# ParsaEsmati/SEA

Measured on AMD Instinct MI355X. Metric: rollout steps/sec (full-context forward, recompute mode) on cylinder_flow-shaped fields, higher is better.
Workload: dtype bf16

## Files before the change

include/sea_hip.h:

```cpp
#ifndef SEA_HIP_H
#define SEA_HIP_H

#include <stddef.h>
#include <stdint.h>

#ifdef __cplusplus
extern "C" {
#endif

#define SEA_ABI_VERSION 8

enum { SEA_F32 = 0, SEA_BF16 = 1 };

enum {
    SEA_OK = 0,
    SEA_EINVAL = -1,
    SEA_ELAUNCH = -2,
    SEA_EUNSUPPORTED = -3
};

int sea_abi_version(void);
const char* sea_last_error(void);
const char* sea_last_form(int* a, int* b);
int sea_struct_sizes(int* out, int cap);
// ... 393 lines not shown
    const float* b3;
    void* mod3;
    int32_t ldw3, ldmod3;
    uint32_t* memo_stamps;
    void* memo_mods;
    const uint32_t* memo_epoch;
    int32_t* memo_count;
    uint32_t* memo_rows;
    int32_t ldmemo, pad_;
} SeaAdalnQkv;
int sea_adaln_qkv(const SeaAdalnQkv* groups, int n_groups, const SeaQkvCommon* common, const SeaGemmGroup* riders, int n_riders, const SeaSiluGroup* silu, int n_silu,
                  const float* silu_c, int silu_M, const SeaIbParams* ib, float eps, int dtype, void* stream);

#define SEA_CHAIN_MAX_PROJ 6
#define SEA_CHAIN_MAX_GROUPS 3
typedef struct {
    const void* att[SEA_XTAIL_MAX_SEG];
    const void* Wp[SEA_XTAIL_MAX_SEG];
    const void* a2;
    const void* W2;
    const float* b2;
    const float* Xin;
    float* X;
    void* Xact;
    int32_t n_seg, ldatt, ldwp, lda2, ldw2, ldxin, ldx, ldxact;
    int32_t M, D, E, has_down, n_proj;
    float bias_scale;
    SeaGemmNormGroup down;
    SeaQkvGroup proj[SEA_CHAIN_MAX_PROJ];
    uint32_t* tile_stamps;
    const float* tile_cond;
    const uint32_t* tile_epoch;
    int32_t* tile_count;
    int32_t tile_sets, pad_;
} SeaRowChain;

int sea_row_chain(const SeaRowChain* params, int n_groups, const SeaQkvCommon* common, float eps, int dtype, void* stream);
struct SeaIbParams_;
int sea_row_chain_riders(const SeaRowChain* params, int n_groups, const SeaQkvCommon* common, const SeaGemmGroup* riders, int n_riders, int tile0, int n_tiles,
                         const struct SeaIbParams_* ib, float eps, int dtype, void* stream);

enum { SEA_OP_GEMM = 1, SEA_OP_QKV = 2, SEA_OP_ATTN = 3, SEA_OP_NORM = 4, SEA_OP_SILU = 5, SEA_OP_IB = 6, SEA_OP_CONVERT = 8, SEA_OP_GEMM_NORM = 9, SEA_OP_XTAIL = 10, SEA_OP_MLP1 = 11, SEA_OP_MLP2 = 13, SEA_OP_GEMM_FEW = 14, SEA_OP_QKV_FEW = 15, SEA_OP_CHAIN = 16, SEA_OP_ADALN = 17, SEA_OP_MLPB = 18, SEA_OP_AQKV = 19, SEA_OP_SPLITK = 20 };
// ... 336 lines not shown
```

sea_amd/_native.py:

```python
from __future__ import annotations

import ctypes as C
import os
from typing import Optional

import torch

_HERE = os.path.dirname(os.path.abspath(__file__))
LIB_PATH = os.path.join(_HERE, "csrc", "libsea_hip.so")

SEA_F32, SEA_BF16 = 0, 1
ABI_VERSION = 8
MAX_GROUPS = 16
CTL_GRAD_NORM, CTL_CLIP, CTL_INV_BC1, CTL_INV_SQRT_BC2, CTL_APPLIED, CTL_STEP, CTL_SKIPPED, CTL_CLIPPED, CTL_WORDS = range(9)
MAX_ATTN_PROBLEMS = 8
MAX_NORM_GROUPS = 16
MAX_SILU_GROUPS = 24

_vp, _i32, _i64, _f32 = C.c_void_p, C.c_int32, C.c_int64, C.c_float


class SeaDropout(C.Structure):
    _fields_ = [("seed", C.c_uint32), ("stream", C.c_uint32), ("thr", _i32), ("mode", _i32)]

# ... 101 lines not shown

XTAIL_MAX_SEG = 4
XTAIL_MAX_GROUPS = 4
MAX_SILU_IB = 4


class SeaExchangeTail(C.Structure):
    _fields_ = [("att", _vp * XTAIL_MAX_SEG), ("Wp", _vp * XTAIL_MAX_SEG), ("Wup", _vp), ("bup", _vp), ("X", _vp), ("Xact", _vp),
                ("n_seg", _i32), ("ldatt", _i32), ("ldwp", _i32), ("ldwup", _i32), ("ldx", _i32), ("ldxact", _i32),
                ("M", _i32), ("D", _i32), ("E", _i32), ("has_down", _i32), ("bias_scale", _f32),
                ("down", SeaGemmNormGroup)]


CHAIN_MAX_PROJ = 6
CHAIN_MAX_GROUPS = 3
CHAIN_MAX_RIDERS = 8


class SeaRowChain(C.Structure):
    _fields_ = [("att", _vp * XTAIL_MAX_SEG), ("Wp", _vp * XTAIL_MAX_SEG), ("a2", _vp), ("W2", _vp), ("b2", _vp), ("Xin", _vp), ("X", _vp), ("Xact", _vp),
                ("n_seg", _i32), ("ldatt", _i32), ("ldwp", _i32), ("lda2", _i32), ("ldw2", _i32), ("ldxin", _i32), ("ldx", _i32), ("ldxact", _i32),
                ("M", _i32), ("D", _i32), ("E", _i32), ("has_down", _i32), ("n_proj", _i32), ("bias_scale", _f32),
                ("down", SeaGemmNormGroup), ("proj", SeaQkvGroup * CHAIN_MAX_PROJ),
                ("tile_stamps", _vp), ("tile_cond", _vp), ("tile_epoch", _vp), ("tile_count", _vp), ("tile_sets", _i32), ("pad_", _i32)]


MAX_ADALN_GROUPS = 16


class SeaAdalnGroup(C.Structure):
    _fields_ = [("A", _vp), ("W", _vp), ("bias", _vp), ("X", _vp), ("gamma", _vp), ("beta", _vp), ("Yact", _vp), ("Y32", _vp), ("mean", _vp), ("rstd", _vp),
                ("lda", _i32), ("ldw", _i32), ("ldx", _i32), ("ldyact", _i32), ("ldy32", _i32), ("M", _i32), ("d", _i32), ("K", _i32)]


MAX_SPLITK_GROUPS = 8


# ... 403 lines not shown
```

sea_amd/csrc/chain.hip:

```cpp
#include "norm_epilogue.hpp"
#include "gemm_tile.hpp"
#include "ib_rows.hpp"
#include <stdlib.h>

struct ChainLaunch {
    SeaRowChain p[SEA_CHAIN_MAX_GROUPS];
    SeaQkvCommon c;
    float eps;
    int n_groups;
    unsigned long long* stamps;
    ChainRiderPod rg[SEA_CHAIN_MAX_RIDERS];
    int n_riders, rider_t0, rider_n, ib_wgs;
    SeaIbParams ib;
};
static_assert(sizeof(ChainLaunch) <= 4096, "kernel arguments of sea_row_chain");

static unsigned long long* g_chain_stamps = nullptr;
extern "C" void sea_chain_debug_stamps(unsigned long long* buf) { g_chain_stamps = buf; }

template <int D, int E, int MI>
struct ChainCfg {
    static constexpr int BM = 16 * MI, BKB = 128, BK = 64;
    static constexpr int KTD = D / BK, KTE = E / BK;
    static constexpr int AT_BYTES = BM * E * 2;
// ... 131 lines not shown
    float* Y32;
    void* Yact;
    float* mean;
    float* rstd;
};

template <int D, int E, int MI>
__global__ __launch_bounds__(256) void row_chain_kernel(const ChainLaunch L) {
    using T = __bf16;
    using C = ChainCfg<D, E, MI>;
    constexpr int BM = C::BM, KTD = C::KTD, KTE = C::KTE, NI1 = C::NI1, NI2 = C::NI2, NI3 = C::NI3, NI4 = C::NI4, SMAX = C::SMAX;
    constexpr int A_KTS = BM * 128;
    extern __shared__ __attribute__((aligned(16))) char smem[];
    const int tid = threadIdx.x, lane = tid & 63, wave = tid >> 6;
    const int r = lane & 15, g = lane >> 4;
    if ((int)blockIdx.y == L.n_groups) {
        const int x = blockIdx.x;
        if (x < L.rider_n) {
            const int tile = L.rider_t0 + x;
            int gi = 0;
            while (gi + 1 < L.n_riders && tile >= L.rg[gi + 1].tile_start) ++gi;
            const ChainRiderPod& R = L.rg[gi];
            ChainRiderGroup G;
            G.A = R.A; G.W = R.W; G.bias = R.bias; G.Cact = R.Cact;
            G.lda = R.lda; G.ldw = R.ldw; G.ldcact = R.ldcact; G.M = R.M; G.N = R.N; G.K = R.K;
            const int t = tile - R.tile_start;
            const int tiles_n = (R.N + 127) / 128;
            const int tm = t / tiles_n, tn = t % tiles_n;
            uint32_t* tst = L.p[0].tile_stamps;
            uint32_t t_c[2] = {0u, 0u}, t_e = 0u;
            int t_row[2] = {-1, -1};
// ... 22 lines not shown
                __syncthreads();
            }
            gemm_tile_body<T, 128, 128, true, true, false>(G, tm, tn, smem, 0);
#pragma unroll
            for (int i = 0; i < 2; ++i)
                if (tst != nullptr && t_row[i] >= 0) reinterpret_cast<uint2*>(tst)[t_row[i]] = make_uint2(t_c[i], t_e);
        } else if (x < L.rider_n + L.ib_wgs) {
            const int row0 = (x - L.rider_n) * 64 + wave * 16;
            for (int i = 0; i < 16; ++i) {
                const int row = row0 + i;
                if (row < L.ib.M) ib_store_row(L.ib, L.ib.c[row], row, lane);
            }
        }
        return;
    }
    ChainParams pl;
    {
        const uint32_t* raw = reinterpret_cast<const uint32_t*>(&L.p[0]) + (size_t)blockIdx.y * (sizeof(SeaRowChain) / 4);
#pragma unroll
        for (int k = 0; k < 4; ++k) {
            const int dw = k * 64 + lane;
            pl.v[k] = dw < (int)(sizeof(SeaRowChain) / 4) ? raw[dw] : 0u;
        }
    }
    const int M = CP_I32(M), S = CP_I32(n_seg);
    const int m0 = blockIdx.x * BM;
    if (m0 >= M) return;
    unsigned long long* stp = L.stamps != nullptr ? L.stamps + (size_t)(blockIdx.y * gridDim.x + blockIdx.x) * 16 : nullptr;
    int stn = 0;
    auto stamp = [&]() {
        if (stp != nullptr && tid == 0 && stn < 16) stp[stn] = wall_clock64();
        ++stn;
    };
    stamp();
    char* AT = smem;
    char* YT = AT + C::AT_BYTES;
    char* WA = YT + C::YT_BYTES;
    char* WB = WA + C::WH_BYTES;
    float* s_rope = reinterpret_cast<float*>(WB + C::WH_BYTES);
    float* s_bias = reinterpret_cast<float*>(reinterpret_cast<char*>(s_rope) + C::ROPE_BYTES);
    float* red = reinterpret_cast<float*>(reinterpret_cast<char*>(s_bias) + C::BIAS_BYTES);
    const unsigned lds0 = __builtin_amdgcn_readfirstlane((unsigned)(uintptr_t)smem);
    const unsigned at_l = lds0, wa_l = lds0 + C::AT_BYTES + C::YT_BYTES, wb_l = wa_l + C::WH_BYTES;
    const int wv = __builtin_amdgcn_readfirstlane(wave);
    const T* W2 = CP_PTR(const T*, W2);
    const int ldw2 = CP_I32(ldw2);
    const bool has_down = CP_I32(has_down) != 0;
    const int n_proj = has_down ? CP_I32(n_proj) : 0;
    const T* Wd = CP_PTR(const T*, down.W);
    const int ldwd = CP_I32(down.ldw);

    if (S > 0) {
        const int ldatt = CP_I32(ldatt), ldwp = CP_I32(ldwp);
#pragma unroll
        for (int s = 0; s < SMAX; ++s) {
            if (s < S) {
                const T* att = reinterpret_cast<const T*>(cp_dyn_u64(pl, CP_DW(att) + 2 * s));
                const T* Wp = reinterpret_cast<const T*>(cp_dyn_u64(pl, CP_DW(Wp) + 2 * s));
                chain_dma_a(att, ldatt, m0, M - 1, BM, KTD, at_l + (unsigned)(s * KTD * A_KTS), wv, lane);
                chain_dma_w(Wp, ldwp, D, 0, KTD, wa_l + (unsigned)(s * D * D * 2), wv, lane);
            }
        }
        chain_dma_w(W2, ldw2, E, 0, KTD, wb_l, wv, lane);
// ... 20 lines not shown
    for (int j = 0; j < NI2; ++j) {
        const int n = wave * (E / 4) + j * 16 + g * 4;
#pragma unroll
        for (int q = 0; q < 4; ++q) bv2[j][q] = 0.f;
        if (b2 != nullptr) load4(b2 + n, bv2[j]);
#pragma unroll
        for (int i = 0; i < MI; ++i) load4(Xin + (int64_t)mrow[i] * ldxin + n, rv2[i][j]);
    }
    ChainNormGroup<D, E> Gd;
    Gd.M = M;
    Gd.bias = CP_PTR(const float*, down.bias);
    Gd.mod = CP_PTR(const void*, down.mod);
    Gd.ldmod = CP_I32(down.ldmod);
    Gd.gamma = CP_PTR(const float*, down.gamma);
    Gd.beta = CP_PTR(const float*, down.beta);
    Gd.Y32 = CP_PTR(float*, down.Y32);
    Gd.ldy32 = CP_I32(down.ldy32);
    Gd.Yact = CP_PTR(void*, down.Yact);
    Gd.ldyact = CP_I32(down.ldyact);
    Gd.mean = CP_PTR(float*, down.mean);
    Gd.rstd = CP_PTR(float*, down.rstd);
    NormEpilogue<T, NI3, true, true, true> epi3[MI];
    if (has_down) {
#pragma unroll
        for (int i = 0; i < MI; ++i) epi3[i].prefetch(Gd, mrow[i], wave * (D / 4), g);
    }
    const int hd = L.c.hd, hd2 = hd >> 1, Tlen = L.c.T, pos0 = L.c.pos0;
    if (n_proj > 0) {
        for (int idx = tid; idx < BM * hd2; idx += 256) {
            const int i = idx / hd2, k = idx - i * hd2;
            int m = m0 + i;
            m = m < M ? m : M - 1;
            const int t = m % Tlen;
            const float2 cs = reinterpret_cast<const float2*>(L.c.rope)[(int64_t)(pos0 + t) * hd2 + k];
            reinterpret_cast<float2*>(s_rope)[idx] = cs;
        }
        int boff = 0;
        for (int e = 0; e < n_proj; ++e) {
            const int base = CP_DW(proj) + e * (int)(sizeof(SeaQkvGroup) / 4);
            const float* bias = reinterpret_cast<const float*>(cp_dyn_u64(pl, base + QK_DW(bias)));
            const int N = (int)cp_dyn_u32(pl, base + QK_DW(N));
            for (int n = tid; n < N; n += 256) s_bias[boff + n] = bias != nullptr ? bias[n] : 0.f;
            boff += N;
        }
    }
#pragma unroll
    for (int j = 0; j < NI2; ++j)
#pragma unroll
        for (int q = 0; q < 4; ++q) {
            touch(bv2[j][q]);
#pragma unroll
            for (int i = 0; i < MI; ++i) touch(rv2[i][j][q]);
        }
// ... 49 lines not shown
                const int kk = wave * (D / 4) + j * 16 + g * 4;
                store4(reinterpret_cast<T*>(YT + (kk >> 6) * A_KTS + (i * 16 + r) * 128 + ((((kk & 63) >> 3) ^ (r & 7)) << 4) + (kk & 7) * 2), gsum[i][j][0], gsum[i][j][1], gsum[i][j][2],
                       gsum[i][j][3]);
            }
        lds_barrier();
        if (has_down) chain_dma_w(Wd, ldwd, D, 0, KTE, wa_l, wv, lane);
        chain_mma<MI, NI2>(YT, A_KTS, WB, E * 128, wave * (E / 4), KTD, NI2, r, g, acc2);
    } else {
        chain_mma<MI, NI2>(AT, A_KTS, WA, E * 128, wave * (E / 4), KTE / 2, NI2, r, g, acc2);
        lds_barrier();
        if (has_down) chain_dma_w(Wd, ldwd, D, 0, KTE, wa_l, wv, lane);
        chain_mma<MI, NI2>(AT + (KTE / 2) * A_KTS, A_KTS, WB, E * 128, wave * (E / 4), KTE / 2, NI2, r, g, acc2);
    }
    lds_barrier();
    stamp();
    int e_next = 0;
    auto burst = [&](unsigned half_l, int& e_lo, int& e_hi) {
        e_lo = e_next;
        int bytes = 0;
        while (e_next < n_proj) {
            const int base = CP_DW(proj) + e_next * (int)(sizeof(SeaQkvGroup) / 4);
            const int N = (int)cp_dyn_u32(pl, base + QK_DW(N));
            if (bytes + N * D * 2 > C::WH_BYTES) break;
            chain_dma_w(reinterpret_cast<const T*>(cp_dyn_u64(pl, base + QK_DW(W))), (int)cp_dyn_u32(pl, base + QK_DW(ldw)), N, 0, KTD, half_l + (unsigned)bytes, wv, lane);
            bytes += N * D * 2;
            ++e_next;
        }
        e_hi = e_next;
    };
    int b_lo[2] = {0, 0}, b_hi[2] = {0, 0};
    if (n_proj > 0) burst(wb_l, b_lo[0], b_hi[0]);
    float v2[MI][NI2][4];
#pragma unroll
    for (int i = 0; i < MI; ++i)
#pragma unroll
        for (int j = 0; j < NI2; ++j) {
            const int n = wave * (E / 4) + j * 16 + g * 4;
#pragma unroll
            for (int q = 0; q < 4; ++q) v2[i][j][q] = acc2[i][j][q] + bv2[j][q] * bias_scale + rv2[i][j][q];
            store4(reinterpret_cast<T*>(AT + (n >> 6) * A_KTS + (i * 16 + r) * 128 + ((((n & 63) >> 3) ^ (r & 7)) << 4) + (n & 7) * 2), v2[i][j][0], v2[i][j][1], v2[i][j][2], v2[i][j][3]);
        }
    asm volatile("s_waitcnt vmcnt(0)" ::: "memory");
    stamp();
    {
        float* X = CP_PTR(float*, X);
        T* Xact = CP_PTR(T*, Xact);
        const int ldx = CP_I32(ldx), ldxact = CP_I32(ldxact);
#pragma unroll
        for (int i = 0; i < MI; ++i) {
            if (!mok[i]) continue;
            float* xr_ = X + (int64_t)(m0 + i * 16 + r) * ldx + wave * (E / 4) + g * 4;
            T* xa_ = Xact != nullptr ? Xact + (int64_t)(m0 + i * 16 + r) * ldxact + wave * (E / 4) + g * 4 : nullptr;
#pragma unroll
            for (int j = 0; j < NI2; ++j) {
                store4(xr_ + j * 16, v2[i][j][0], v2[i][j][1], v2[i][j][2], v2[i][j][3]);
                if (xa_ != nullptr) store4(xa_ + j * 16, v2[i][j][0], v2[i][j][1], v2[i][j][2], v2[i][j][3]);
            }
        }
    }
    stamp();
    if (!has_down) return;
    lds_barrier();
    {
        f32x4 acc3[MI][NI3];
#pragma unroll
        for (int i = 0; i < MI; ++i)
#pragma unroll
            for (int j = 0; j < NI3; ++j) acc3[i][j] = f32x4{0.f, 0.f, 0.f, 0.f};
        chain_mma<MI, NI3>(AT, A_KTS, WA, D * 128, wave * (D / 4), KTE, NI3, r, g, acc3);
#pragma unroll
        for (int i = 0; i < MI; ++i)
            epi3[i].finish(Gd, acc3[i], m0 + i * 16 + r, wave * (D / 4), r, g, wave, L.eps, red + i * 128, n_proj > 0 ? YT + i * 16 * 128 : nullptr, A_KTS);
    }
    stamp();
    if (n_proj == 0) return;
    const int Hh = L.c.H, cap = L.c.cap, Ea = Hh * hd;
    const int hd_sh = 31 - __builtin_clz((unsigned)hd);
    uint32_t offq[MI], offk[MI], offv[MI];
#pragma unroll
    for (int i = 0; i < MI; ++i) {
        const int b_ = mrow[i] / Tlen;
        const int t_ = mrow[i] - b_ * Tlen;
        offq[i] = (uint32_t)((b_ * Hh * Tlen + t_) << hd_sh);
        offk[i] = (uint32_t)((b_ * Hh * cap + pos0 + t_) << hd_sh);
        offv[i] = (uint32_t)(b_ * Hh * hd * cap + pos0 + t_);
    }
    const float q_scale = L.c.q_scale;
    int cur = 0;
    int boff = 0;
    for (;;) {
// ... 129 lines not shown
        R.lda = G.lda; R.ldw = G.ldw; R.ldcact = G.ldcact; R.M = G.M; R.N = G.N; R.K = G.K;
        R.tile_start = rider_total;
        rider_total += ((G.M + 127) / 128) * ((G.N + 127) / 128);
    }
    SEA_REQUIRE(tile0 + n_tiles <= rider_total, "sea_row_chain_riders: tiles [%d, %d) of %d", tile0, tile0 + n_tiles, rider_total);
    L.n_riders = n_riders; L.rider_t0 = tile0; L.rider_n = n_tiles;
    if (ib != nullptr) {
        SEA_REQUIRE(ib->X[0] && ib->c && ib->w1 && ib->M >= 1 && ib->E >= 4 && ib->E % 4 == 0 && ib->ldx >= ib->E && ib->mode >= 0 && ib->mode <= 2 &&
                        (ib->mode != 0 || (ib->b1 && ib->lnw && ib->lnb && ib->w2 && ib->b2 && ib->h >= 1 && ib->h <= 64)),
                    "sea_row_chain_riders: bad info-bottleneck rider");
        L.ib = *ib;
        L.ib_wgs = (ib->M + 63) / 64;
    }
    const int D = params[0].D, E = params[0].E;
    int m_max = 0, any_proj = 0;
    for (int gi = 0; gi < n_groups; ++gi) {
        const SeaRowChain& P = params[gi];
        const bool shape_ok = (P.D == 128 && P.E == 256) || (P.D == 64 && P.E == 128);
        if (dtype != SEA_BF16 || !shape_ok || P.n_seg < 0 || P.n_seg * P.D > P.E) {
            sea_set_error("sea_row_chain: unsupported dtype / shape (dtype=%d D=%d E=%d n_seg=%d): bf16, (D,E) in {(128,256),(64,128)}, n_seg*D <= E", dtype, P.D, P.E, P.n_seg);
            return SEA_EUNSUPPORTED;
        }
        SEA_REQUIRE(P.D == D && P.E == E, "sea_row_chain[%d]: the groups of a launch share their widths", gi);
        SEA_REQUIRE(P.M >= 1 && P.W2 && P.Xin && P.X && sea_aligned16(P.W2) && sea_aligned16(P.b2) && sea_aligned16(P.Xin) && sea_aligned16(P.X) && sea_aligned16(P.Xact),
                    "sea_row_chain[%d]: null / misaligned pointer", gi);
        const int K2 = P.n_seg > 0 ? P.D : P.E;
        SEA_REQUIRE(P.ldw2 % 8 == 0 && P.ldw2 >= K2 && P.ldxin % 4 == 0 && P.ldxin >= P.E && P.ldx % 4 == 0 && P.ldx >= P.E && (!P.Xact || (P.ldxact % 4 == 0 && P.ldxact >= P.E)),
                    "sea_row_chain[%d]: bad strides", gi);
        if (P.n_seg == 0) SEA_REQUIRE(P.a2 && sea_aligned16(P.a2) && P.lda2 % 8 == 0 && P.lda2 >= P.E, "sea_row_chain[%d]: a2: null / misaligned / short rows", gi);
        else SEA_REQUIRE(P.ldatt % 8 == 0 && P.ldatt >= P.D && P.ldwp % 8 == 0 && P.ldwp >= P.D, "sea_row_chain[%d]: bad segment strides", gi);
// ... 17 lines not shown
            const SeaQkvGroup& Q = P.proj[e];
            SEA_REQUIRE(common != nullptr, "sea_row_chain: projections need the SeaQkvCommon");
            const int Ea = common->H * common->hd;
            SEA_REQUIRE(Q.W && sea_aligned16(Q.W) && sea_aligned16(Q.bias) && Q.ldw % 8 == 0 && Q.ldw >= P.D && Q.K == P.D && (Q.N == P.D / 2 || Q.N == P.D || Q.N == 2 * P.D) && Q.N % 64 == 0,
                        "sea_row_chain[%d]: projection %d: W [N, D] with N in {D, 2D} (multiples of 64), K = D (N=%d K=%d ldw=%d)", gi, e, Q.N, Q.K, Q.ldw);
            SEA_REQUIRE((Q.N == P.D && Q.col0 == 0) || (Q.N == 2 * P.D && Q.col0 == P.D), "sea_row_chain[%d]: projection %d: a q entry (N = D, col0 = 0) or a k | v entry (N = 2 D, col0 = D), not N=%d col0=%d", gi, e, Q.N, Q.col0);
            SEA_REQUIRE(Q.col0 >= 0 && Q.col0 % 16 == 0 && Q.col0 + Q.N <= 3 * Ea && Ea == P.D, "sea_row_chain[%d]: projection %d: columns [%d,%d) outside [0,%d) / H hd != D", gi, e, Q.col0, Q.col0 + Q.N, 3 * Ea);
            const bool hasq = Q.col0 < Ea, hask = Q.col0 < 2 * Ea && Q.col0 + Q.N > Ea, hasv = Q.col0 + Q.N > 2 * Ea;
            SEA_REQUIRE((!hasq || Q.Qout) && (!hask || Q.Kout) && (!hasv || Q.Vtout) && sea_aligned16(Q.Qout) && sea_aligned16(Q.Kout) && sea_aligned16(Q.Vtout) && sea_aligned16(Q.Vout),
                        "sea_row_chain[%d]: projection %d: missing / misaligned output pointer", gi, e);
            nsum += Q.N;
            any_proj = 1;
        }
        SEA_REQUIRE(nsum * 4 <= 4096, "sea_row_chain[%d]: the projections' output columns sum to %d (at most 1024)", gi, nsum);
        m_max = P.M > m_max ? P.M : m_max;
    }
    if (any_proj) {
        const SeaQkvCommon& c = *common;
        if (c.hd < 16 || (c.hd & (c.hd - 1)) != 0) {
            sea_set_error("sea_row_chain: unsupported head dim %d (a power of two >= 16: a 16-column block of a projection lies inside one head)", c.hd);
            return SEA_EUNSUPPORTED;
        }
        SEA_REQUIRE(c.rope != nullptr && c.H >= 1 && c.hd >= 4 && c.hd % 4 == 0 && c.T >= 1 && c.pos0 >= 0 && c.cap >= c.pos0 + c.T && m_max % c.T == 0,
                    "sea_row_chain: bad common H=%d hd=%d T=%d pos0=%d cap=%d (M=%d)", c.H, c.hd, c.T, c.pos0, c.cap, m_max);
        SEA_REQUIRE((int64_t)(m_max / c.T + 1) * c.H * c.cap * c.hd < ((int64_t)1 << 31) && (int64_t)(c.pos0 + c.T) * (c.hd / 2) < ((int64_t)1 << 30),
                    "sea_row_chain: attention tensors too large for 32-bit element offsets");
        L.c = c;
    }
    const int forced = sea_tune("chain_rows", 0);
    int mi = ((m_max + 15) / 16) * n_groups <= 256 ? 1 : 2;
    if (forced == 16) mi = 1;
    if (forced == 32) mi = 2;
    if (any_proj && 16 * mi * (L.c.hd / 2) * 8 > 2048) {
        if (mi == 2 && 16 * (L.c.hd / 2) * 8 <= 2048) mi = 1;
        else {
            sea_set_error("sea_row_chain: head dim %d: the rotary rows of a workgroup do not fit their LDS block", L.c.hd);
            return SEA_EUNSUPPORTED;
        }
    }
    hipStream_t s = static_cast<hipStream_t>(stream);
    const int chain_x = (m_max + 16 * mi - 1) / (16 * mi), rider_x = L.rider_n + L.ib_wgs;
    const dim3 grid(chain_x > rider_x ? chain_x : rider_x, n_groups + (rider_x > 0 ? 1 : 0));
    constexpr int rider_lds = GemmMainloop<__bf16, 128, 128>::DMA_LDS_BYTES;
#define LAUNCH_CH(DD, EE, MM)                                                                                   \
    do {                                                                                                        \
        constexpr int own_ = ChainCfg<DD, EE, MM>::LDS_BYTES;                                                   \
        constexpr int max_ = own_ > rider_lds ? own_ : rider_lds;                                               \
        static int once = set_lds_chain(row_chain_kernel<DD, EE, MM>, max_);                                    \
        (void)once;                                                                                             \
        row_chain_kernel<DD, EE, MM><<<grid, dim3(256), (L.rider_n > 0 ? max_ : own_), s>>>(L);                 \
    } while (0)
    if (L.p[0].tile_stamps != nullptr && L.rider_n > 0) {
        const SeaRowChain& P0 = L.p[0];
        SEA_REQUIRE(P0.tile_cond && P0.tile_epoch && P0.tile_sets >= rider_total && ((uintptr_t)P0.tile_stamps & 7) == 0 && ((uintptr_t)P0.tile_cond & 3) == 0 &&
                        ((uintptr_t)P0.tile_epoch & 3) == 0 && ((uintptr_t)P0.tile_count & 3) == 0,
                    "sea_row_chain_riders: tile memo: null / misaligned pointer, or %d stamp sets for %d tiles", P0.tile_sets, rider_total);
        for (int i = 1; i < n_riders; ++i) SEA_REQUIRE(riders[i].M == riders[0].M, "sea_row_chain_riders: tile memo: the rider groups share their rows (one condition per row)");
        if (sea_tune("memo_count", 0) == 0) L.p[0].tile_count = nullptr;
    } else {
        L.p[0].tile_stamps = nullptr;
    }
    if (D == 128) { if (mi == 1) LAUNCH_CH(128, 256, 1); else LAUNCH_CH(128, 256, 2); }
    else { if (mi == 1) LAUNCH_CH(64, 128, 1); else LAUNCH_CH(64, 128, 2); }
#undef LAUNCH_CH
    SEA_CHECK_LAUNCH("sea_row_chain");
    sea_note_form(mi == 1 ? "chain.rows16" : "chain.rows32", L.rider_n, L.ib_wgs);
    return SEA_OK;
}
```

sea_amd/engine.py:

```python
from __future__ import annotations

import os

import ctypes as C
import re
from typing import Dict, List, Optional, Tuple

import torch

from . import _native as N
from . import _switches
from . import ops
from . import ptrcheck
from .plan_forms import INFERENCE, resolve_forms

_QKV = re.compile(r"^(.*\.)(k|q|v)\.(weight|bias)$")
_QKV_RANK = {("q", "weight"): 0, ("k", "weight"): 1, ("v", "weight"): 2, ("q", "bias"): 3, ("k", "bias"): 4, ("v", "bias"): 5}


_BIND_KEYS = {"X_is_x": ("_x_patches", "X"), "R_is_x": ("_x_patches", "R"), "Xin_is_x": ("_x_patches", "Xin"), "Y_is_out": ("_out_patches", "Y32"),
              "dY_is_dout": ("_dout_patches", "dY")}


KV_NO_POOL = ("sea_amd: the KV-cache rollout does not cover exchange_mode='pool' (its sinusoidal positions are relative to the window); "
              "use the recompute rollout")
KV_NO_IB_ATTENTION = ("sea_amd: the KV-cache rollout does not cover ib_addition_mode='attention' (every row attends to the info-bottleneck rows "
                      "of ALL positions of the window, later ones included: rows already produced change as the window grows); use the recompute rollout")
KV_NO_SRC_LEN = "sea_amd: the KV-cache rollout is exact only for src_len == 0; use the recompute rollout (rollout(..., mode='recompute'))"

# ... 588 lines not shown
            nd_old = [self._buf(M, D) for _ in range(F)]
            nd_new = [self._buf(M, D) for _ in range(F)]
            Qc = [self._buf(B, H, T, hd_c) for _ in range(max(F - 1, 1))]
            Qc2 = [[self._buf(B, H, T, hd_c) for _ in range(F - 1)] for _ in range(F)] if chain else None
            Kc = [[[self._buf(B, H, cap, hd_c, zero=True) for _ in range(F)] for _ in range(F)] for _ in range(self.L)]
            Vc = [[[self._buf(B, H, hd_c, cap, zero=True) for _ in range(F)] for _ in range(F)] for _ in range(self.L)]
            att_c = [self._buf(M, D) for _ in range(max(F - 1, 1))]
            gp = self._buf(max(F - 1, 1), M, D)
        pad = fm.hidden_pad
        hbuf = [self._buf(M, S + pad)[:, :S] for _ in range(F)]
        hg = [self._buf(M, S + pad)[:, :S] for _ in range(F)]
        self.ws = dict(xr=xr, xa=xa, n_e=n_e, att_e=att_e, hbuf=hbuf, hg=hg)
        self.kv = dict(Ks=Ks, Vs=Vs, Kc=(Kc if xmode == "sea" else None), Vc=(Vc if xmode == "sea" else None))

        xm = [self._buf(M, E) for _ in range(F)] if lanes else xa
        first = True
        for l in range(self.L):
            pre = f"blocks.{l}."
            last = l == self.L - 1
            if first and not eng.model.add_info_after_cross and (has_ib or ib_attn or concat):
                for i in range(F):
                    rec = _Rec(L.sea_convert_f32_to_act, [None, FE, xr[i].data_ptr(), E, M, Eo, N.SEA_F32], "x.copy")
                    self._x_patches.append((rec.args, 0, i * Eo * 4))
                    self.records.append(rec)
                first = False
            if concat:
                if self._zero_ib is None:
                    self._zero_ib = self._buf(M, self.ib_dim, dtype=f32, zero=True)
                for i in range(F):
                    self._cur.append(self._rec(L.sea_convert_f32_to_act, [self._zero_ib.data_ptr(), self.ib_dim, xr[i][:, Eo:].data_ptr(), E, M, self.ib_dim, N.SEA_F32],
# ... 48 lines not shown
            if chain:
                groups = []
                for i in range(F):
                    proj = []
                    for s_, j in enumerate([j for j in range(F) if j != i]):
                        ca = f"{pre}cross_attn.{i}.{j}."
                        proj.append(dict(W=P.act(ca + "q.weight"), bias=P.f32_vec(ca + "q.bias"), col0=0, Q=Qc2[i][s_]))
                    for a in range(i):
                        ca = f"{pre}cross_attn.{a}.{i}."
                        proj.append(dict(W=P.act(ca + "k.weight", 2 * D), bias=P.f32_vec(ca + "k.bias", 2 * D), col0=D, K=Kc[l][a][i], Vt=Vc[l][a][i]))
                    g = dict(a2=att_e[i], W2=P.act(f"{pre}attn.self.{i}.projection.weight"), Xin=xr[i], X=xr[i], proj=proj,
                             down=dict(W=P.act(f"{pre}cross_down.{i}.weight"), bias=P.f32_vec(f"{pre}cross_down.{i}.bias"), **self._norm_params(f"{pre}ln_cross.{i}.")))
                    if first:
                        g.update(ldxin=FE, Xin_is_x=i * Eo * 4)
                    groups.append(g)
                self._chain(groups, rope_c, hd_c, "self.out_proj_down_qkv")
            else:
                (self._gemm_few if few else self._gemm)(groups, "self.out_proj")
            first = False
            if not cond_joined:
                self._join(1)
                cond_joined = True
            if xmode == "addition":
                ndall = self._buf(F, M, D)
                self._down_norm(pre, range(F), xa, dn, ndall, "add")
                sg = self._buf(M, D)
                self._gemm([dict(A=ndall[0], W=eng.eye(D), n_seg=F, a_seg_stride=M * D, Cact=sg, act=1)], "add.sum_gelu")
                self._gemm([dict(A=sg, W=P.act(f"{pre}cross_up.{i}.weight"), bias=P.f32_vec(f"{pre}cross_up.{i}.bias"), R=xr[i], C32=xr[i])
                            for i in range(F)], "add.up")
            if xmode == "pool":
                FD = F * D
# ... 42 lines not shown
                              bias_scale=float(F - 1), n_seg=F - 1, a_seg_stride=M * D, R=xr[i], C32=xr[i], Cact=(xa[i] if i < F - 1 else None))
                    (self._gemm_few if F == 2 else self._gemm)([up], f"cross{i}.up_sum")
                    if i < F - 1:
                        self._gemm_few([dict(A=xa[i], W=P.act(f"{pre}cross_down.{i}.weight"), bias=P.f32_vec(f"{pre}cross_down.{i}.bias"), C32=dn[i])], f"cross{i}.down_new")
            elif F > 1 and xmode == "sea" and chain:
                for i in range(F):
                    others = [j for j in range(F) if j != i]
                    self._attn([dict(Q=Qc2[i][s_], K=Kc[l][i][j], Vt=Vc[l][i][j], O=att_c[s_]) for s_, j in enumerate(others)], hd_c, D, f"cross{i}.attention")
                    proj = []
                    for b_ in range(i + 1, F):
                        ca = f"{pre}cross_attn.{b_}.{i}."
                        proj.append(dict(W=P.act(ca + "k.weight", 2 * D), bias=P.f32_vec(ca + "k.bias", 2 * D), col0=D, K=Kc[l][b_][i], Vt=Vc[l][b_][i]))
                    down = None
                    if i < F - 1:
                        down = dict(W=P.act(f"{pre}cross_down.{i}.weight"), bias=P.f32_vec(f"{pre}cross_down.{i}.bias"), **self._norm_params(f"{pre}ln_cross.{i}."))
                    self._chain([dict(att=[att_c[s_] for s_ in range(len(others))], Wp=[P.act(f"{pre}cross_attn.{i}.{j}.projection.weight") for j in others],
                                      W2=P.act(f"{pre}cross_up.{i}.weight"), b2=P.f32_vec(f"{pre}cross_up.{i}.bias"), bias_scale=float(F - 1), Xin=xr[i], X=xr[i],
                                      down=down, proj=proj)], rope_c, hd_c, f"cross{i}.tail")
            elif F > 1 and xmode == "sea":
                self._down_norm(pre, range(F), xa, dn, nd_old, "cross", "_old")
                for i in range(F):
                    others = [j for j in range(F) if j != i]
                    qkv_groups, probs, proj_groups = [], [], []
                    for s, j in enumerate(others):
                        src = nd_new[j] if j < i else nd_old[j]
                        ca = f"{pre}cross_attn.{i}.{j}."
                        qkv_groups.append(dict(A=nd_old[i], W=P.act(ca + "q.weight"), bias=P.f32_vec(ca + "q.bias"), col0=0, Q=Qc[s]))
                        qkv_groups.append(dict(A=src, W=P.act(ca + "k.weight", 2 * D), bias=P.f32_vec(ca + "k.bias", 2 * D), col0=D,
                                               K=Kc[l][i][j], Vt=Vc[l][i][j]))
                        probs.append(dict(Q=Qc[s], K=Kc[l][i][j], Vt=Vc[l][i][j], O=att_c[s]))
                        proj_groups.append(dict(A=att_c[s], W=P.act(ca + "projection.weight"), Cact=gp[s], act=1))
                    self._qkv(qkv_groups, rope_c, hd_c, f"cross{i}.qkv_rope")
                    self._attn(probs, hd_c, D, f"cross{i}.attention")
# ... 453 lines not shown
            for k, r in enumerate(recs):
                rc = r.fn(*r.args, stream)
                if rc != 0:
                    N.check(rc, r.name)
                evs[k + 1].record()
            torch.cuda.synchronize()
            for k in range(n):
                tot[k] += evs[k].elapsed_time(evs[k + 1])
        return [(r.name, t / iters) for r, t in zip(recs, tot)]


def blk_pe(eng: "TemporalEngine", layer: int) -> torch.Tensor:
    return eng.model.blocks[layer].pos_encoder.pe[0].to(device=eng.device, dtype=torch.float32)


def _require_gpu(device: torch.device) -> None:
    if device.type != "cuda":
        raise RuntimeError("sea_amd: TemporalModel runs only on an MI355X (no CPU fallback)")


class TemporalEngine:

    def __init__(self, model: torch.nn.Module, device: torch.device, act_dtype: torch.dtype):
        N.lib()
        _require_gpu(device)
        m = model
        self.ib_mode = {"mlp": 0, "linear": 1, "fourier": 2}.get(m.ib_scale_mode.lower(), -1)
        if (m.exchange_mode not in ("sea", "addition", "simple", "pool") or self.ib_mode < 0 or m.ib_addition_mode.lower() not in ("add", "none", "attention", "concat")
                or (self.ib_mode == 0 and m.ib_mlp_layers != 1) or m.ib_num != 1 or (self.ib_mode != 0 and m.embed_dim % 8 and m.ib_addition_mode.lower() != "concat")):
            raise NotImplementedError(
# ... 278 lines not shown
```

sea_amd/ops.py:

```python
from __future__ import annotations

import ctypes as C
import math
from typing import Dict, Optional, Sequence

import torch

from . import _native as N


def _mat(t: torch.Tensor, name: str) -> torch.Tensor:
    N.require_gpu(t, name)
    if t.dim() != 2 or t.stride(1) != 1:
        raise ValueError(f"{name}: need a 2-D tensor with unit inner stride, got shape {tuple(t.shape)} strides {t.stride()}")
    return t


def fill_gemm_group(g: N.SeaGemmGroup, A, W, bias=None, R=None, C32=None, Cact=None, n_seg=1, a_seg_stride=0, act=0,
                    bias_scale=1.0, M=None, N_=None, K=None, Z=None, silu=None, drop=None, ldr=None, ldc32=None) -> None:
    if silu is not None:
        c = silu.get("c")
        g.silu_c, g.silu_w1, g.silu_b1 = N.ptr(c), silu["w1"].data_ptr(), silu["b1"].data_ptr()
        A, R, Z, n_seg, a_seg_stride, act = None, None, None, 1, 0, 0
        M = c.numel() if M is None else M
# ... 302 lines not shown
            fill_silu_group(g, gd["w1"], gd["b1"], gd["Hid"])
    ibp = None
    if ib is not None:
        ibp = N.SeaIbParams()
        fill_ib_params(ibp, **ib)
    N.check(N.lib().sea_adaln_qkv(arr, len(groups), C.byref(c), rarr, len(riders), sarr, len(silu), (silu_c.data_ptr() if silu_c is not None else None),
                                  (silu_c.numel() if silu_c is not None else 0), (C.byref(ibp) if ibp is not None else None), eps, N.dtype_code(dtype), N.stream_ptr()),
            "sea_adaln_qkv")


def row_chain_supported(dtype: torch.dtype, D: int, E: int, n_seg: int, hd: int) -> bool:
    return dtype == torch.bfloat16 and (D, E) in ((128, 256), (64, 128)) and 0 <= n_seg and n_seg * D <= E and hd in (16, 32)


def fill_row_chain(P: N.SeaRowChain, W2, Xin, X, att: Sequence[torch.Tensor] = (), Wp: Sequence[torch.Tensor] = (), a2=None, b2=None, bias_scale: float = 1.0, Xact=None,
                   down: Optional[Dict] = None, proj: Sequence[Dict] = (), ldxin: Optional[int] = None, tile_memo: Optional[Dict] = None) -> None:
    if tile_memo is not None:
        st = tile_memo["stamps"]
        if st.dtype != torch.int32 or st.dim() != 3 or tuple(st.shape[1:]) != (128, 2) or not st.is_contiguous():
            raise ValueError(f"row_chain tile memo: stamps {tuple(st.shape)} {st.dtype}: int32 [tiles, 128, 2], one set per rider tile")
        P.tile_stamps, P.tile_sets = st.data_ptr(), st.shape[0]
        P.tile_cond, P.tile_epoch, P.tile_count = N.ptr(tile_memo.get("cond")), tile_memo["epoch"].data_ptr(), N.ptr(tile_memo.get("count"))
    for s_, a in enumerate(att):
        P.att[s_] = a.data_ptr()
        P.Wp[s_] = Wp[s_].data_ptr()
    P.n_seg = len(att)
    if att:
        P.ldatt, P.ldwp = att[0].stride(0), Wp[0].stride(0)
    if a2 is not None:
        P.a2, P.lda2 = a2.data_ptr(), a2.stride(0)
    P.W2, P.ldw2, P.b2, P.bias_scale = W2.data_ptr(), W2.stride(0), N.ptr(b2), bias_scale
# ... 1458 lines not shown
```

sea_amd/plan_forms.py:

```python
from __future__ import annotations

from dataclasses import dataclass, field
from typing import Dict, Optional, Tuple

import torch

from . import _native as N
from . import _switches
from . import ops

INFERENCE, TRAINING, CONDITION = "inference", "training", "condition"


@dataclass(frozen=True)
class PlanForms:
    lanes: bool
    split_cond: bool
    chain: bool
    riders: bool
    rider_caps: Optional[Tuple[int, ...]]
    gen_a: bool
    fold_ib: bool
    hoist_ib: bool
    ib_rows_here: bool
# ... 2 lines not shown
    few_fold_ln: bool
    hidden_pad: int
    front_chain: bool
    front3: bool
    adaln_front: bool
    front_big: bool
    mlp_fc1: bool
    mlp_norm_in: bool
    mlp_block: bool
    mlp_fc2_proj: bool
    down_norm: bool
    proj_norm: bool
    splitk: bool
    cond_memo: bool = field(default=False, compare=False)
    rider_memo: bool = field(default=False, compare=False)

    @property
    def one_launch_front(self) -> bool:
        return self.front_big or self.front_chain


def resolve_forms(model, B: int, T: int, mode: str, dt: torch.dtype, kind: str = INFERENCE, hoisted: bool = False, hoisted_ib: bool = False,
                  plan_switches: Optional[Dict[str, str]] = None, kv_switches: Optional[Dict[str, str]] = None) -> PlanForms:
    assert kind in (INFERENCE, TRAINING, CONDITION)
    sw = (_switches.parse("SEA_PLAN") if plan_switches is None else plan_switches).get
    kvsw = (_switches.parse("SEA_KV") if kv_switches is None else kv_switches).get
    inference = kind == INFERENCE
    F, H, L = model.num_variables, model.n_heads, model.num_layers
    Eo, E, D, S, M = model.embed_dim, model.internal_embed_dim, model.down_dim, model.mlp_hidden, B * T
    xmode, ib_add = model.exchange_mode, model.ib_addition_mode.lower()
    has_ib, ib_attn, concat = ib_add == "add", ib_add == "attention", ib_add == "concat"
    after, adaln = bool(model.add_info_after_cross), model.LN_type.lower() == "adaln"

    lane_mode = sw("lanes", "auto") if inference and xmode == "sea" and has_ib else "none"
# ... 32 lines not shown
    w1, wn, w2 = sw("mlp1", "auto"), sw("mlpnorm", "auto"), sw("mlp2", "auto")
    mlp_fc1 = inference and w1 != "0" and (w1 == "1" or M >= 1024) and mlp_ok
    mlp_norm_in = mlp_fc1 and (wn == "1" or (wn == "auto" and M <= 4096))
    mlp_block = (mlp_fc1 and inference and (w2 == "1" or (w2 == "auto" and 1024 <= M)) and mlp_ok and Eo == E and sw("mlpblock", "1") != "0")
    if mlp_block:
        mlp_norm_in = mlp_norm_in or (M > 4096 and wn != "0")
    mlp_fc2_proj = not mlp_block and inference and (w2 == "1" or (w2 == "auto" and 1024 <= M <= 4096)) and mlp_ok and Eo == E

    return PlanForms(
        lanes=lanes, split_cond=split_cond, chain=chain, riders=riders, rider_caps=(tuple(int(v) for v in caps.split(":")) if caps else None),
        gen_a=gen_a, fold_ib=fold_ib or hoist_ib, hoist_ib=hoist_ib, ib_rows_here=ib_rows_here, xtail=xtail, few=few, few_fold_ln=S <= 8192,
        hidden_pad=(64 if inference and S % 1024 == 0 else 0), front_chain=front_chain, front3=front3, adaln_front=adaln_front, front_big=front_big,
        mlp_fc1=mlp_fc1, mlp_norm_in=mlp_norm_in, mlp_block=mlp_block, mlp_fc2_proj=mlp_fc2_proj,
        down_norm=(fuse_norm if inference else kind == TRAINING and sw("norm", "1") != "0") and D <= 256 and D % 16 == 0,
        proj_norm=fuse_norm and Eo <= 256 and Eo % 16 == 0 and Eo == E and sw("projnorm", "1") != "0", splitk=sw("splitk", "1") != "0",
        cond_memo=front_chain and riders and sw("cond_memo", "1") != "0", rider_memo=front_chain and riders and sw("rider_memo", "1") != "0")
```

sea_amd/ptrcheck.py:

```python
from __future__ import annotations

import ctypes as C
import os
from typing import Iterable, Iterator, List, Optional, Tuple

import torch

from . import _native as N

_HOST_STRUCTS = (N.SeaLaunchRec, N.SeaStepPatch)


def always() -> bool:
    return os.environ.get("SEA_CHECK_PTRS", "0") == "1"


class Ranges:

    def __init__(self) -> None:
        self._r: List[Tuple[int, int, str]] = []

    def add_tensor(self, t: Optional[torch.Tensor], label: str) -> None:
        if t is None or not isinstance(t, torch.Tensor) or not t.is_cuda or t.numel() == 0:
            return
# ... 234 lines not shown
            roots.append(r.keep)
        for root in roots:
            for st in _walk_structs(root):
                for path, p in iter_pointers(st, type(st).__name__):
                    n += 1
                    if ranges.find(p) is None:
                        raise RuntimeError(f"sea_amd pointer audit ({what}): launch '{r.name}': {path} = {p:#x} lies in no buffer this plan knows "
                                           "(stale address, unpatched field or a tensor that was freed)")
                for field, p, nbytes in _extents(st, esz):
                    if not p:
                        continue
                    hit = ranges.find(p)
                    if hit is not None and nbytes > 0 and p + nbytes > hit[1]:
                        raise RuntimeError(f"sea_amd pointer audit ({what}): launch '{r.name}': {type(st).__name__}.{field} = {p:#x} + {nbytes} bytes runs "
                                           f"{p + nbytes - hit[1]} bytes past the end of its buffer ({hit[2]})")
        for field, p, nbytes in _raw_extents(r, esz):
            hit = ranges.find(p)
            if hit is not None and nbytes > 0 and p + nbytes > hit[1]:
                raise RuntimeError(f"sea_amd pointer audit ({what}): launch '{r.name}': argument {field} = {p:#x} + {nbytes} bytes runs "
                                   f"{p + nbytes - hit[1]} bytes past the end of its buffer ({hit[2]})")
        for a in r.args:
            if isinstance(a, int) and a >= (1 << 32) and ranges.find(a) is None and r.fn is not None and r.name not in ("",):
                if _looks_like_device_pointer(a):
                    raise RuntimeError(f"sea_amd pointer audit ({what}): launch '{r.name}': raw argument {a:#x} lies in no buffer this plan knows")
    return n


def _looks_like_device_pointer(a: int) -> bool:
    return a >= (1 << 40) and a % 4 == 0
```

Measured before the change: 5650.

## Split row-chain projection bursts across sibling workgroup rows to fill CUs

Adds a per-group split factor to the row-chain kernel. Each group's QKV projection bursts are divided among several virtual grid rows. Siblings recompute the shared out-proj and down-norm front, but only the primary writes the residual and norm outputs, so the grid can cover more CUs when the tile count is small. This duplicates front work and needs a separate X buffer per split group (ping-pong allocation), with host and pointer-audit checks that X and Xin do not overlap.

```diff
diff --git a/include/sea_hip.h b/include/sea_hip.h
--- a/include/sea_hip.h
+++ b/include/sea_hip.h
@@ -431,6 +431,7 @@
 
 #define SEA_CHAIN_MAX_PROJ 6
 #define SEA_CHAIN_MAX_GROUPS 3
+#define SEA_CHAIN_MAX_SPLIT 3
 typedef struct {
     const void* att[SEA_XTAIL_MAX_SEG];
     const void* Wp[SEA_XTAIL_MAX_SEG];
@@ -443,6 +444,7 @@
     int32_t n_seg, ldatt, ldwp, lda2, ldw2, ldxin, ldx, ldxact;
     int32_t M, D, E, has_down, n_proj;
     float bias_scale;
+    int32_t split, pad0_;
     SeaGemmNormGroup down;
     SeaQkvGroup proj[SEA_CHAIN_MAX_PROJ];
     uint32_t* tile_stamps;
diff --git a/sea_amd/_native.py b/sea_amd/_native.py
--- a/sea_amd/_native.py
+++ b/sea_amd/_native.py
@@ -139,6 +139,7 @@
 
 CHAIN_MAX_PROJ = 6
 CHAIN_MAX_GROUPS = 3
+CHAIN_MAX_SPLIT = 3
 CHAIN_MAX_RIDERS = 8
 
 
@@ -146,6 +147,7 @@
     _fields_ = [("att", _vp * XTAIL_MAX_SEG), ("Wp", _vp * XTAIL_MAX_SEG), ("a2", _vp), ("W2", _vp), ("b2", _vp), ("Xin", _vp), ("X", _vp), ("Xact", _vp),
                 ("n_seg", _i32), ("ldatt", _i32), ("ldwp", _i32), ("lda2", _i32), ("ldw2", _i32), ("ldxin", _i32), ("ldx", _i32), ("ldxact", _i32),
                 ("M", _i32), ("D", _i32), ("E", _i32), ("has_down", _i32), ("n_proj", _i32), ("bias_scale", _f32),
+                ("split", _i32), ("pad0_", _i32),
                 ("down", SeaGemmNormGroup), ("proj", SeaQkvGroup * CHAIN_MAX_PROJ),
                 ("tile_stamps", _vp), ("tile_cond", _vp), ("tile_epoch", _vp), ("tile_count", _vp), ("tile_sets", _i32), ("pad_", _i32)]
 
diff --git a/sea_amd/csrc/chain.hip b/sea_amd/csrc/chain.hip
--- a/sea_amd/csrc/chain.hip
+++ b/sea_amd/csrc/chain.hip
@@ -3,11 +3,14 @@
 #include "ib_rows.hpp"
 #include <stdlib.h>
 
+#define SEA_CHAIN_MAX_VROWS (SEA_CHAIN_MAX_GROUPS * SEA_CHAIN_MAX_SPLIT)
 struct ChainLaunch {
     SeaRowChain p[SEA_CHAIN_MAX_GROUPS];
     SeaQkvCommon c;
     float eps;
     int n_groups;
+    int n_vrows;
+    uint32_t vrow[SEA_CHAIN_MAX_VROWS];
     unsigned long long* stamps;
     ChainRiderPod rg[SEA_CHAIN_MAX_RIDERS];
     int n_riders, rider_t0, rider_n, ib_wgs;
@@ -169,7 +172,7 @@
     extern __shared__ __attribute__((aligned(16))) char smem[];
     const int tid = threadIdx.x, lane = tid & 63, wave = tid >> 6;
     const int r = lane & 15, g = lane >> 4;
-    if ((int)blockIdx.y == L.n_groups) {
+    if ((int)blockIdx.y == L.n_vrows) {
         const int x = blockIdx.x;
         if (x < L.rider_n) {
             const int tile = L.rider_t0 + x;
@@ -222,9 +225,12 @@
         }
         return;
     }
+    const uint32_t vrow = L.vrow[blockIdx.y];
+    const bool primary = ((vrow >> 8) & 0xffu) == 0u;
+    const int e_first = (int)((vrow >> 16) & 0xffu);
     ChainParams pl;
     {
-        const uint32_t* raw = reinterpret_cast<const uint32_t*>(&L.p[0]) + (size_t)blockIdx.y * (sizeof(SeaRowChain) / 4);
+        const uint32_t* raw = reinterpret_cast<const uint32_t*>(&L.p[0]) + (size_t)(vrow & 0xffu) * (sizeof(SeaRowChain) / 4);
 #pragma unroll
         for (int k = 0; k < 4; ++k) {
             const int dw = k * 64 + lane;
@@ -254,7 +260,7 @@
     const T* W2 = CP_PTR(const T*, W2);
     const int ldw2 = CP_I32(ldw2);
     const bool has_down = CP_I32(has_down) != 0;
-    const int n_proj = has_down ? CP_I32(n_proj) : 0;
+    const int n_proj = has_down ? (int)(vrow >> 24) : 0;
     const T* Wd = CP_PTR(const T*, down.W);
     const int ldwd = CP_I32(down.ldw);
 
@@ -305,19 +311,19 @@
     Gd.ldmod = CP_I32(down.ldmod);
     Gd.gamma = CP_PTR(const float*, down.gamma);
     Gd.beta = CP_PTR(const float*, down.beta);
-    Gd.Y32 = CP_PTR(float*, down.Y32);
+    Gd.Y32 = primary ? CP_PTR(float*, down.Y32) : nullptr;
     Gd.ldy32 = CP_I32(down.ldy32);
-    Gd.Yact = CP_PTR(void*, down.Yact);
+    Gd.Yact = primary ? CP_PTR(void*, down.Yact) : nullptr;
     Gd.ldyact = CP_I32(down.ldyact);
-    Gd.mean = CP_PTR(float*, down.mean);
-    Gd.rstd = CP_PTR(float*, down.rstd);
+    Gd.mean = primary ? CP_PTR(float*, down.mean) : nullptr;
+    Gd.rstd = primary ? CP_PTR(float*, down.rstd) : nullptr;
     NormEpilogue<T, NI3, true, true, true> epi3[MI];
     if (has_down) {
 #pragma unroll
         for (int i = 0; i < MI; ++i) epi3[i].prefetch(Gd, mrow[i], wave * (D / 4), g);
     }
     const int hd = L.c.hd, hd2 = hd >> 1, Tlen = L.c.T, pos0 = L.c.pos0;
-    if (n_proj > 0) {
+    if (n_proj > e_first) {
         for (int idx = tid; idx < BM * hd2; idx += 256) {
             const int i = idx / hd2, k = idx - i * hd2;
             int m = m0 + i;
@@ -327,7 +333,7 @@
             reinterpret_cast<float2*>(s_rope)[idx] = cs;
         }
         int boff = 0;
-        for (int e = 0; e < n_proj; ++e) {
+        for (int e = e_first; e < n_proj; ++e) {
             const int base = CP_DW(proj) + e * (int)(sizeof(SeaQkvGroup) / 4);
             const float* bias = reinterpret_cast<const float*>(cp_dyn_u64(pl, base + QK_DW(bias)));
             const int N = (int)cp_dyn_u32(pl, base + QK_DW(N));
@@ -407,7 +413,7 @@
     }
     lds_barrier();
     stamp();
-    int e_next = 0;
+    int e_next = e_first;
     auto burst = [&](unsigned half_l, int& e_lo, int& e_hi) {
         e_lo = e_next;
         int bytes = 0;
@@ -422,7 +428,7 @@
         e_hi = e_next;
     };
     int b_lo[2] = {0, 0}, b_hi[2] = {0, 0};
-    if (n_proj > 0) burst(wb_l, b_lo[0], b_hi[0]);
+    if (n_proj > e_first) burst(wb_l, b_lo[0], b_hi[0]);
     float v2[MI][NI2][4];
 #pragma unroll
     for (int i = 0; i < MI; ++i)
@@ -435,7 +441,7 @@
         }
     asm volatile("s_waitcnt vmcnt(0)" ::: "memory");
     stamp();
-    {
+    if (primary) {
         float* X = CP_PTR(float*, X);
         T* Xact = CP_PTR(T*, Xact);
         const int ldx = CP_I32(ldx), ldxact = CP_I32(ldxact);
@@ -463,10 +469,10 @@
         chain_mma<MI, NI3>(AT, A_KTS, WA, D * 128, wave * (D / 4), KTE, NI3, r, g, acc3);
 #pragma unroll
         for (int i = 0; i < MI; ++i)
-            epi3[i].finish(Gd, acc3[i], m0 + i * 16 + r, wave * (D / 4), r, g, wave, L.eps, red + i * 128, n_proj > 0 ? YT + i * 16 * 128 : nullptr, A_KTS);
+            epi3[i].finish(Gd, acc3[i], m0 + i * 16 + r, wave * (D / 4), r, g, wave, L.eps, red + i * 128, n_proj > e_first ? YT + i * 16 * 128 : nullptr, A_KTS);
     }
     stamp();
-    if (n_proj == 0) return;
+    if (n_proj == e_first) return;
     const int Hh = L.c.H, cap = L.c.cap, Ea = Hh * hd;
     const int hd_sh = 31 - __builtin_clz((unsigned)hd);
     uint32_t offq[MI], offk[MI], offv[MI];
@@ -626,6 +632,7 @@
     }
     const int D = params[0].D, E = params[0].E;
     int m_max = 0, any_proj = 0;
+    int split_max = 1, split_asked = 0, n_vrows = 0;
     for (int gi = 0; gi < n_groups; ++gi) {
         const SeaRowChain& P = params[gi];
         const bool shape_ok = (P.D == 128 && P.E == 256) || (P.D == 64 && P.E == 128);
@@ -673,7 +680,35 @@
         }
         SEA_REQUIRE(nsum * 4 <= 4096, "sea_row_chain[%d]: the projections' output columns sum to %d (at most 1024)", gi, nsum);
         m_max = P.M > m_max ? P.M : m_max;
-    }
+        SEA_REQUIRE(P.split >= 0 && P.split <= SEA_CHAIN_MAX_SPLIT, "sea_row_chain[%d]: split=%d (0 .. %d)", gi, P.split, SEA_CHAIN_MAX_SPLIT);
+        int burst_end[SEA_CHAIN_MAX_PROJ], n_bursts = 0;
+        for (int e = 0, bytes = 0; e < P.n_proj; ++e) {
+            const int eb = P.proj[e].N * P.D * 2;
+            if (n_bursts == 0 || bytes + eb > P.E * P.D * 2) {
+                ++n_bursts;
+                bytes = 0;
+            }
+            bytes += eb;
+            burst_end[n_bursts - 1] = e + 1;
+        }
+        int sp = P.split > 1 ? P.split : 1;
+        split_asked |= P.split > 1 ? 1 : 0;
+        sp = sp > n_bursts ? (n_bursts > 0 ? n_bursts : 1) : sp;
+        if (sp > 1) {
+            const char *xi = reinterpret_cast<const char*>(P.Xin), *xo = reinterpret_cast<const char*>(P.X);
+            const int64_t xi_bytes = ((int64_t)(P.M - 1) * P.ldxin + P.E) * 4, xo_bytes = ((int64_t)(P.M - 1) * P.ldx + P.E) * 4;
+            SEA_REQUIRE(xi + xi_bytes <= xo || xo + xo_bytes <= xi,
+                        "sea_row_chain[%d]: split=%d needs X and Xin in distinct memory (a sibling may read its residual rows after sibling 0 has stored the updated ones)", gi, P.split);
+        }
+        for (int k = 0, b0 = 0; k < sp; ++k) {
+            const int nb = n_bursts / sp + (k >= sp - n_bursts % sp ? 1 : 0);
+            const int e_lo = sp == 1 ? 0 : (b0 == 0 ? 0 : burst_end[b0 - 1]), e_hi = sp == 1 ? P.n_proj : burst_end[b0 + nb - 1];
+            L.vrow[n_vrows++] = (uint32_t)gi | (uint32_t)k << 8 | (uint32_t)e_lo << 16 | (uint32_t)e_hi << 24;
+            b0 += nb;
+        }
+        split_max = sp > split_max ? sp : split_max;
+    }
+    L.n_vrows = n_vrows;
     if (any_proj) {
         const SeaQkvCommon& c = *common;
         if (c.hd < 16 || (c.hd & (c.hd - 1)) != 0) {
@@ -687,7 +722,7 @@
         L.c = c;
     }
     const int forced = sea_tune("chain_rows", 0);
-    int mi = ((m_max + 15) / 16) * n_groups <= 256 ? 1 : 2;
+    int mi = ((m_max + 15) / 16) * n_vrows <= 256 ? 1 : 2;
     if (forced == 16) mi = 1;
     if (forced == 32) mi = 2;
     if (any_proj && 16 * mi * (L.c.hd / 2) * 8 > 2048) {
@@ -699,7 +734,7 @@
     }
     hipStream_t s = static_cast<hipStream_t>(stream);
     const int chain_x = (m_max + 16 * mi - 1) / (16 * mi), rider_x = L.rider_n + L.ib_wgs;
-    const dim3 grid(chain_x > rider_x ? chain_x : rider_x, n_groups + (rider_x > 0 ? 1 : 0));
+    const dim3 grid(chain_x > rider_x ? chain_x : rider_x, n_vrows + (rider_x > 0 ? 1 : 0));
     constexpr int rider_lds = GemmMainloop<__bf16, 128, 128>::DMA_LDS_BYTES;
 #define LAUNCH_CH(DD, EE, MM)                                                                                   \
     do {                                                                                                        \
@@ -723,6 +758,7 @@
     else { if (mi == 1) LAUNCH_CH(64, 128, 1); else LAUNCH_CH(64, 128, 2); }
 #undef LAUNCH_CH
     SEA_CHECK_LAUNCH("sea_row_chain");
-    sea_note_form(mi == 1 ? "chain.rows16" : "chain.rows32", L.rider_n, L.ib_wgs);
+    if (split_asked) sea_note_form("chain.split", split_max, 0);
+    else sea_note_form(mi == 1 ? "chain.rows16" : "chain.rows32", L.rider_n, L.ib_wgs);
     return SEA_OK;
 }
diff --git a/sea_amd/engine.py b/sea_amd/engine.py
--- a/sea_amd/engine.py
+++ b/sea_amd/engine.py
@@ -12,7 +12,7 @@
 from . import _switches
 from . import ops
 from . import ptrcheck
-from .plan_forms import INFERENCE, resolve_forms
+from .plan_forms import CHAIN_SPLIT_GROWTH, INFERENCE, chain_bursts, chain_splits, resolve_forms
 
 _QKV = re.compile(r"^(.*\.)(k|q|v)\.(weight|bias)$")
 _QKV_RANK = {("q", "weight"): 0, ("k", "weight"): 1, ("v", "weight"): 2, ("q", "bias"): 3, ("k", "bias"): 4, ("v", "bias"): 5}
@@ -631,6 +631,30 @@
         self.kv = dict(Ks=Ks, Vs=Vs, Kc=(Kc if xmode == "sea" else None), Vc=(Vc if xmode == "sea" else None))
 
         xm = [self._buf(M, E) for _ in range(F)] if lanes else xa
+        cus = device_cu_count() if fm.chain_split else 0
+        spare: List[torch.Tensor] = []
+
+        def split_chain(groups: List[dict], fields) -> List[dict]:
+            if not fm.chain_split or cus <= 0:
+                return groups
+            n, t16 = len(groups), (M + 15) // 16
+            rows = 16 if t16 * n <= 256 else 32
+            sp = chain_splits([chain_bursts([q["W"].shape[0] for q in g["proj"]], D, E) for g in groups], [(M + rows - 1) // rows] * n, cus,
+                              max_growth=(None if fm.chain_split_all else CHAIN_SPLIT_GROWTH))
+            if rows == 16 and t16 * sum(sp) > 256:
+                return groups
+            out, freed = [], []
+            for g, i, s_ in zip(groups, fields, sp):
+                if s_ > 1:
+                    g = dict(g, split=s_)
+                    if "Xin_is_x" not in g:
+                        new = spare.pop() if spare else self._buf(M, E, dtype=f32)
+                        freed.append(xr[i])
+                        g["X"] = xr[i] = new
+                out.append(g)
+            spare.extend(freed)
+            return out
+
         first = True
         for l in range(self.L):
             pre = f"blocks.{l}."
@@ -709,7 +733,7 @@
                     if first:
                         g.update(ldxin=FE, Xin_is_x=i * Eo * 4)
                     groups.append(g)
-                self._chain(groups, rope_c, hd_c, "self.out_proj_down_qkv")
+                self._chain(split_chain(groups, range(F)), rope_c, hd_c, "self.out_proj_down_qkv")
             else:
                 (self._gemm_few if few else self._gemm)(groups, "self.out_proj")
             first = False
@@ -782,9 +806,10 @@
                     down = None
                     if i < F - 1:
                         down = dict(W=P.act(f"{pre}cross_down.{i}.weight"), bias=P.f32_vec(f"{pre}cross_down.{i}.bias"), **self._norm_params(f"{pre}ln_cross.{i}."))
-                    self._chain([dict(att=[att_c[s_] for s_ in range(len(others))], Wp=[P.act(f"{pre}cross_attn.{i}.{j}.projection.weight") for j in others],
-                                      W2=P.act(f"{pre}cross_up.{i}.weight"), b2=P.f32_vec(f"{pre}cross_up.{i}.bias"), bias_scale=float(F - 1), Xin=xr[i], X=xr[i],
-                                      down=down, proj=proj)], rope_c, hd_c, f"cross{i}.tail")
+                    tail = dict(att=[att_c[s_] for s_ in range(len(others))], Wp=[P.act(f"{pre}cross_attn.{i}.{j}.projection.weight") for j in others],
+                                W2=P.act(f"{pre}cross_up.{i}.weight"), b2=P.f32_vec(f"{pre}cross_up.{i}.bias"), bias_scale=float(F - 1), Xin=xr[i], X=xr[i],
+                                down=down, proj=proj)
+                    self._chain(split_chain([tail], [i]), rope_c, hd_c, f"cross{i}.tail")
             elif F > 1 and xmode == "sea":
                 self._down_norm(pre, range(F), xa, dn, nd_old, "cross", "_old")
                 for i in range(F):
@@ -1268,6 +1293,11 @@
     return eng.model.blocks[layer].pos_encoder.pe[0].to(device=eng.device, dtype=torch.float32)
 
 
+def device_cu_count() -> int:
+    n = C.c_int(0)
+    return n.value if N.lib().sea_device_info(C.byref(n), None, 0) == 0 else 0
+
+
 def _require_gpu(device: torch.device) -> None:
     if device.type != "cuda":
         raise RuntimeError("sea_amd: TemporalModel runs only on an MI355X (no CPU fallback)")
diff --git a/sea_amd/ops.py b/sea_amd/ops.py
--- a/sea_amd/ops.py
+++ b/sea_amd/ops.py
@@ -340,7 +340,8 @@
 
 
 def fill_row_chain(P: N.SeaRowChain, W2, Xin, X, att: Sequence[torch.Tensor] = (), Wp: Sequence[torch.Tensor] = (), a2=None, b2=None, bias_scale: float = 1.0, Xact=None,
-                   down: Optional[Dict] = None, proj: Sequence[Dict] = (), ldxin: Optional[int] = None, tile_memo: Optional[Dict] = None) -> None:
+                   down: Optional[Dict] = None, proj: Sequence[Dict] = (), ldxin: Optional[int] = None, tile_memo: Optional[Dict] = None, split: int = 1) -> None:
+    P.split = split
     if tile_memo is not None:
         st = tile_memo["stamps"]
         if st.dtype != torch.int32 or st.dim() != 3 or tuple(st.shape[1:]) != (128, 2) or not st.is_contiguous():
diff --git a/sea_amd/plan_forms.py b/sea_amd/plan_forms.py
--- a/sea_amd/plan_forms.py
+++ b/sea_amd/plan_forms.py
@@ -1,7 +1,7 @@
 from __future__ import annotations
 
 from dataclasses import dataclass, field
-from typing import Dict, Optional, Tuple
+from typing import Dict, List, Optional, Sequence, Tuple
 
 import torch
 
@@ -40,10 +40,39 @@
     splitk: bool
     cond_memo: bool = field(default=False, compare=False)
     rider_memo: bool = field(default=False, compare=False)
+    chain_split: bool = field(default=False, compare=False)
+    chain_split_all: bool = field(default=False, compare=False)
 
     @property
     def one_launch_front(self) -> bool:
         return self.front_big or self.front_chain
+
+
+def chain_bursts(widths: Sequence[int], D: int, E: int) -> int:
+    n, used = 0, 0
+    for w in widths:
+        if n == 0 or used + w * D > E * D:
+            n, used = n + 1, 0
+        used += w * D
+    return n
+
+
+CHAIN_SPLIT_GROWTH = 0.5
+
+
+def chain_splits(bursts: Sequence[int], tiles: Sequence[int], cus: int, max_split: int = N.CHAIN_MAX_SPLIT, max_growth: Optional[float] = CHAIN_SPLIT_GROWTH) -> List[int]:
+    splits = [1] * len(bursts)
+    rounds = lambda sp: [-(-b // s) for b, s in zip(bursts, sp)]
+    cap = cus if max_growth is None else min(cus, int(sum(tiles) * (1.0 + max_growth)))
+    while True:
+        now = rounds(splits)
+        worst = max(now, default=0)
+        if worst <= 1:
+            return splits
+        more = [s + 1 if r == worst else s for s, r in zip(splits, now)]
+        if max(more) > max_split or max(rounds(more)) >= worst or sum(t * s for t, s in zip(tiles, more)) > cap:
+            return splits
+        splits = more
 
 
 def resolve_forms(model, B: int, T: int, mode: str, dt: torch.dtype, kind: str = INFERENCE, hoisted: bool = False, hoisted_ib: bool = False,
@@ -106,4 +135,5 @@
         mlp_fc1=mlp_fc1, mlp_norm_in=mlp_norm_in, mlp_block=mlp_block, mlp_fc2_proj=mlp_fc2_proj,
         down_norm=(fuse_norm if inference else kind == TRAINING and sw("norm", "1") != "0") and D <= 256 and D % 16 == 0,
         proj_norm=fuse_norm and Eo <= 256 and Eo % 16 == 0 and Eo == E and sw("projnorm", "1") != "0", splitk=sw("splitk", "1") != "0",
-        cond_memo=front_chain and riders and sw("cond_memo", "1") != "0", rider_memo=front_chain and riders and sw("rider_memo", "1") != "0")
+        cond_memo=front_chain and riders and sw("cond_memo", "1") != "0", rider_memo=front_chain and riders and sw("rider_memo", "1") != "0",
+        chain_split=chain and sw("chain_split", "1") != "0", chain_split_all=chain and sw("chain_split", "1") == "all")
diff --git a/sea_amd/ptrcheck.py b/sea_amd/ptrcheck.py
--- a/sea_amd/ptrcheck.py
+++ b/sea_amd/ptrcheck.py
@@ -272,6 +272,12 @@
                     if hit is not None and nbytes > 0 and p + nbytes > hit[1]:
                         raise RuntimeError(f"sea_amd pointer audit ({what}): launch '{r.name}': {type(st).__name__}.{field} = {p:#x} + {nbytes} bytes runs "
                                            f"{p + nbytes - hit[1]} bytes past the end of its buffer ({hit[2]})")
+                if isinstance(st, N.SeaRowChain) and st.split > 1:
+                    ext = {field: (p, nbytes) for field, p, nbytes in _extents(st, esz) if field in ("Xin", "X")}
+                    (xi, ni), (xo, no) = ext["Xin"], ext["X"]
+                    if xi and xo and xi < xo + no and xo < xi + ni:
+                        raise RuntimeError(f"sea_amd pointer audit ({what}): launch '{r.name}': SeaRowChain.split = {st.split} with X = {xo:#x} + {no} bytes "
+                                           f"overlapping Xin = {xi:#x} + {ni} bytes (a split group needs distinct output rows)")
         for field, p, nbytes in _raw_extents(r, esz):
             hit = ranges.find(p)
             if hit is not None and nbytes > 0 and p + nbytes > hit[1]:
```

Result: faster. 5740, median of 6 (+1.6%).
